# kieranrcampbell/clonealign

Hardware: AMD Instinct MI355X
Metric: ELBO iterations/sec (higher is better)
Workload: dtype f32 variables (contraction: float64 series over gene bins; count-matrix products: int8 MFMA, exact); 1 GPU; synthetic 100000 cells x 5000 genes x 8 clones, K=1, S=1, cell-sharded over 1 GPU(s) (BASELINE.json configs[2]); cells=100000, genes=5000, clones=8, K=1, mc_samples=1, y_storage=u8, y_bytes_per_elem=1, fused_sweep=True, fwd_mfma=True, series_form=True, y_mfma=True, parallelism=single, collective=none, allreduce_doubles_per_train_pass=20764, build_id=9192b4fa1486e0e0

## Files before the change

clonealign_amd/csrc/ca_eng_create.inc:

```

constexpr double CA_ML_STREAM_FIXED_US = 6.6;
constexpr double CA_ML_STREAM_BYTES_PER_US = 5.62e6;
constexpr double CA_ML_MIN_STREAM_US = 45.0;
constexpr int CA_ML_MAX_PER = 4;
struct ca_mom_last_in {
  int slots;
  int n_cu;
  int nb_stream, nb_ovf;
  int ngrp, nred;
  int64_t image_bytes;
};
inline int ca_mom_last_free(const ca_mom_last_in& a) { return std::max(a.slots - a.nb_stream, 0); }
inline int ca_mom_last_free_x(const ca_mom_last_in& a) {
  const int xcd = std::max(a.n_cu / 32, 1);
  return a.slots / xcd - cdiv(a.nb_stream, xcd);
}
inline int ca_mom_last_per(const ca_mom_last_in& a) {
  const int xcd = std::max(a.n_cu / 32, 1), free_x = ca_mom_last_free_x(a);
  if (free_x < 1) return 0;
  return std::max(1, cdiv(a.ngrp, free_x * xcd));
}
inline bool ca_mom_last_pick(const ca_mom_last_in& a) {
  if (a.nb_stream + a.ngrp + a.nred <= a.slots) return false;
  const int per = ca_mom_last_per(a);
// ... 375 lines not shown
                                                 : hipOccupancyMaxActiveBlocksPerMultiprocessor(&per_cu, k_ys_mfma_mom<true>, CA_YM_TB, CA_YS4_LDS_BYTES))
                                 : (h->n_ovf > 0 ? hipOccupancyMaxActiveBlocksPerMultiprocessor(&per_cu, k_ys_mfma_ovf_mom<false>, CA_YM_TB, CA_YS_LDS_BYTES)
                                                 : hipOccupancyMaxActiveBlocksPerMultiprocessor(&per_cu, k_ys_mfma_mom<false>, CA_YM_TB, CA_YS_LDS_BYTES));
    if (oe != hipSuccess) { (void)hipGetLastError(); per_cu = 0; }
    ml.slots = per_cu * h->n_cu; ml.n_cu = h->n_cu;
    ml.nb_stream = h->ys_nrg * h->ys_nseg;
    ml.nb_ovf = h->n_ovf > 0 ? cdiv(Nn, CA_TB) + cdiv(h->n_ovf_chunk, CA_TB / 64) : 0;
    ml.ngrp = h->pws.n_gene_blocks; ml.nred = CA_MOM_NRED;
    ml.image_bytes = h->ys_N64 * h->Gp / (h->ys4 ? 2 : 1);
    h->mom_free_slots = ca_mom_last_free(ml);
    h->mom_last = variantx_on(h, CA_VARX_MOM_LAST, "CA_MOM_LAST_ON") || (variant_on(h, CA_VAR_MOM_LAST, "CA_MOM_LAST") && ca_mom_last_pick(ml));
    if (h->opt.variant_off & CA_VAR_MOM_LAST) h->mom_last = false;
    if (h->mom_last) {
      const int per = ca_mom_last_per(ml);
      h->mom_per = per < 1 ? CA_MOM_PER : std::min(per, CA_ML_MAX_PER);
      h->mom_nred = 2 * CA_MOM_NRED;
      const int lab = (h->opt.reserved[1] & ~0xFF) ? h->opt.reserved[1] >> 8 : 0;
      if (lab & 15) h->mom_per = lab & 15;
      if (lab & 16) h->mom_nred = CA_MOM_NRED;
      h->mom_ovf_first = (lab & 32) != 0;
    }
  }
  h->cell_lean = h->poly && variant_on(h, CA_VAR_CELL_LEAN, "CA_CELL_LEAN");
  h->ride_ok = h->ystore == CA_YSTORE_U8 && K == 1 && D <= 2 && h->fused_ok && !h->c16 && h->fwd_cell && (h->fc_tl == 6 || h->fc_tl == 8 || (h->fc_tl == 2 && h->fc_nbig == 0)) &&
               !h->y_ys && variant_on(h, CA_VAR_Y_RIDE, "CA_Y_RIDE");
  const bool tl1_ok = h->fc_tl == 1 && h->fc_nbig == 0 && !h->c16;
  h->ride_ys = h->y_ys && (!h->ys4 || (h->poly && D == 1 && !h->c16 && !h->s2)) && D <= 2 && h->fused_ok && h->fwd_cell && (h->fc_tl == 6 || tl1_ok || (h->fc_tl == 2 && h->fc_nbig == 0)) &&
               variant_on(h, CA_VAR_Y_RIDE, "CA_Y_RIDE");
  h->yfin_split = h->ride_ys && h->bwd_mfma && h->tail_fuse && variant_on(h, CA_VAR_YFIN_RIDE, "CA_YFIN_RIDE");
  if (h->y_ys && !h->ride_ys) h->async_y = false;
  {
    const int tiles = cdiv(Nn, 16), qb = tiles / std::max(h->n_cu, 1), rb = tiles - qb * h->n_cu;
    h->fwd_bal = h->ride_ys && !h->c16 && !h->s2 && D == 1 && C <= 8 && qb >= 1 && qb <= 6 && h->nk32 >= 96 && h->host_dev && variant_on(h, CA_VAR_FWD_BAL, "CA_FWD_BAL");
    if (h->fwd_bal) {
      h->bal_q = qb; h->bal_r = rb;
      h->bal_nchunk = rb > 0 ? std::min(CA_BAL_MAXCHUNK, h->n_cu / rb) : 0;
      CACK(dalloc(h, &h->bal_xw, std::max<int64_t>(1, (int64_t)rb * h->bal_nchunk * 512)));
    }
  }
  h->s2f = h->s2 && h->fused_ok && h->fwd_cell && (h->fc_tl == 2 || h->fc_tl == 6) && (h->ride_ys || !h->ride_ok) && variant_on(h, CA_VAR_S2_FUSE, "CA_S2_FUSE");
  h->layout_series = h->poly || (h->poly_shape && h->opt.world > 1);
  if (h->layout_series) {
    h->off_y = 3 + C;
    h->off_q = h->off_y + (int64_t)h->Gp * K;
    h->off_x = h->off_q + (int64_t)CA_PL_NB * (CA_PL_R + 2) * 8;
    h->off_g = h->off_x + std::max(h->opt.world, 1);
// ... 93 lines not shown
```

clonealign_amd/csrc/ca_eng_loop.inc:

```
int wait_y(ca_engine* h, bool all) {
  if (all) {
    if (h->y_pending) HIPCK(h, hipStreamWaitEvent(h->stream, h->ev_ydone, 0));
    h->y_pending = false; h->yw_pending = false;
  } else if (h->yw_pending) {
    HIPCK(h, hipStreamWaitEvent(h->stream, h->ev_ywdone, 0));
    h->yw_pending = false;
  }
  return CA_OK;
}

int make_etamax(ca_engine* h) {
  if (h->D > 0) {
    LAUNCH(h, CA_KERNEL_OTHER, hipLaunchKernelGGL(k_vmm_final, dim3(1), dim3(64), 0, h->stream, h->vmm_part, h->vmm, h->ngblk, h->D));
    LAUNCH(h, CA_KERNEL_OTHER, hipLaunchKernelGGL(k_etamax, dim3(cdiv(h->N, CA_TB)), dim3(CA_TB), 0, h->stream, h->F, h->vmm, h->etamax2, h->N, h->D));
  }
  h->em_stale = false;
  return CA_OK;
}
int ensure_etamax(ca_engine* h) {
  if (!h->em_stale) return CA_OK;
  return make_etamax(h);
}

int refresh_derived(ca_engine* h) {
// ... 722 lines not shown
    }
    h->ys_defer_next = h->y_ys && !h->ycache_valid && h->opt.reserved[1] != 3;
    const int yrc = ensure_ycache(h);
    const bool mom_left = h->mom_args != nullptr;
    h->mom_args = nullptr;
    CACK(yrc);
    if (mom_left) { h->err = "internal: the series form's moments were to ride on a count-matrix stream launch that was not made"; return CA_ERR_STATE; }
    h->ys_defer_next = false;
    ca_yfin_args yfin_ride;
    const bool yfin_rides = h->yfin_pending;
    if (yfin_rides) { yfin_ride = yfin_args(h, h->ys_nrg, h->ys_nseg); h->yfin_pending = false; }
    if (moments_aside) HIPCK(h, hipStreamWaitEvent(h->stream, h->ev_poly1, 0));
    CACK(prof_begin(h, CA_KERNEL_FWD));
    ca_small_args ltail = no_small_args();
    const bool sh = is_sharded(h) && h->tail_fuse && yfin_rides;
    if (sh) {
      ltail = small_args(h, h->gene_part, 0, 0.f, nullptr, true);
      ltail.ncblk = h->pws.n_cell_blocks;
      if (h->K > 0) { ltail.yw_part = h->yw_part; ltail.n_yw = h->n_yw; }
      ltail.reduce_only = 1; ltail.host_out = nullptr;
    }
    e = ca_poly_cells(h->stream, &h->pws, h->N, h->C, h->K, &cp, h->alpha_u, h->cell_part, h->dFpart, yfin_rides ? &yfin_ride : nullptr,
                      sh ? &ltail : nullptr, h->poly_xmax_ready ? h->poly_xpart : nullptr, (int)cdiv(h->N, CA_TB), h->F, sh ? h->red + h->off_x : nullptr,
                      h->opt.rank, std::max(h->opt.world, 1), h->cell_lean);
    h->mon_tail_local = sh;
    if (sh) { h->poly_xslot_pending = true; h->poly_xglob_steps = -1; }
    HIPCK(h, e);
    CACK(prof_end(h));
    cell_blocks = h->pws.n_cell_blocks;
    h->poly_fresh = true;
  } else
  if (h->fwd_cell && ride && h->ride_ys) {
    cell_blocks = h->ncblk_f;
    CACK(ys_quant(h));
    ca_ysride_args ya;
    memset(&ya, 0, sizeof(ya));
    ya.Ys = h->Ys; ya.io = ys_io(h); ya.F = h->F; ya.V = h->V; ya.Df = h->D;
    ya.Gp = h->Gp; ya.RS = h->ys_RS; ya.nb_main = h->ys_nrg * h->ys_nseg; ya.nb_y = ya.nb_main;
    ya.ovf = ys_ovf(h);
    ya.nb_y += ya.ovf.nb_rows + ya.ovf.nb_chunks;
    if (h->fwd_bal && !s2f) {
      ca_bal_args ba;
      memset(&ba, 0, sizeof(ba));
      ba.nb = h->n_cu; ba.r = h->bal_r; ba.nchunk = h->bal_nchunk; ba.xw = h->bal_xw;
      cell_blocks = h->n_cu;
      if (++h->bal_tag == 0u) h->bal_tag = 1u;
      ba.tag = h->bal_tag;
// ... 188 lines not shown
```

clonealign_amd/csrc/ca_eng_state.inc:

```
namespace {

thread_local std::string g_last_error;

typedef struct { char internal[128]; } ca_nccl_uid;
typedef void* ca_nccl_comm;
struct RcclApi {
  void* lib = nullptr;
  int (*GetUniqueId)(ca_nccl_uid*) = nullptr;
  int (*CommInitRank)(ca_nccl_comm*, int, ca_nccl_uid, int) = nullptr;
  int (*CommDestroy)(ca_nccl_comm) = nullptr;
  int (*AllReduce)(const void*, void*, size_t, int, int, ca_nccl_comm, hipStream_t) = nullptr;
  const char* (*GetErrorString)(int) = nullptr;
  std::string err;
  bool load() {
    if (lib) return true;
    const char* cands[] = {getenv("CLONEALIGN_RCCL_LIB"), "librccl.so.1", "librccl.so", "/opt/rocm/lib/librccl.so.1",
                           "/opt/rocm/lib/librccl.so"};
    for (const char* c : cands) {
      if (!c || !*c) continue;
      lib = dlopen(c, RTLD_NOW | RTLD_LOCAL);
      if (lib) break;
    }
    if (!lib) { err = std::string("cannot dlopen librccl: ") + dlerror(); return false; }
    GetUniqueId = (decltype(GetUniqueId))dlsym(lib, "ncclGetUniqueId");
// ... 85 lines not shown
  float* eps_dev = nullptr; int64_t eps_cap = 0;
  float *mu32 = nullptr, *Mb = nullptr, *Vs = nullptr, *vmm = nullptr, *vmm_part = nullptr, *etamax2 = nullptr;
  double* gene_part = nullptr; int ngblk = 0;
  float *Zpart = nullptr, *coef = nullptr; double* scratch = nullptr;
  double* cell_part = nullptr; int ncblk = 0;
  float *gpart = nullptr, *dFpart = nullptr; int gsplit = 1, gchunk = 0, csplit = 1; int64_t cchunk = 0; int RG = 4, ntile = 0;
  float *YWpart = nullptr, *YTpart = nullptr, *YW = nullptr; double* ytpsi = nullptr;
  double* red = nullptr; int64_t red_n = 0, off_g = 0, off_y = 0;
  int64_t off_q = 0, off_x = 0;
  bool poly_shape = false, layout_series = false;
  bool mon_tail_local = false;
  bool poly_xslot_pending = false;
  int poly_xglob_steps = -1;
  double* elbo_dev = nullptr; int64_t elbo_cap = 0; double* terms_dev = nullptr;
  double* host_pinned = nullptr;
  bool ycache_valid = false, sums_global = false, sums_started = false;
  std::vector<double> mu_part;
  bool fused_ok = false, look_valid = false; int64_t look_slot = 0; int frow = 8;
  bool carry = false, carry_builtin = false; std::vector<float> carry_eps;
  int64_t n_series = 0, n_series_fallback = 0;
  double *poly_ring = nullptr, *poly_ring_dev = nullptr; uint64_t poly_seq = 0, poly_seq_base = 1, adam_steps = 0, poly_steps_at[16] = {};
  bool mom_ride = false; unsigned mom_tag = 0; const ca_pm_args* mom_args = nullptr;
  bool mom_last = false, mom_ovf_first = false; int mom_free_slots = 0, mom_per = CA_MOM_PER, mom_nred = CA_MOM_NRED;
  bool cell_lean = false;
  bool poly = false, poly_side = false, poly_y_defer = false, poly_fresh = false, poly_df = false ; ca_poly_ws pws; float* poly_zero = nullptr; unsigned char* poly_mem = nullptr;
  float *Mb2 = nullptr, *mu32B = nullptr, *Zpart2 = nullptr; double* gene_partB = nullptr;
  bool y_defer = false;
  bool ride_ok = false;
  bool ride_ys = false;
  bool fold_gsum = false, fold_now = false;
  int64_t hint_A = -1, hint_B = -1, pre_A = -1, pre_B = -1;
  bool pre_valid = false, pre_ok = true, pair_elbo = true;
  double* ee_partB = nullptr;
  double *gene_part_alt = nullptr, *gene_partB_alt = nullptr;
  bool bwd_ready = false; int64_t bwd_slot = -1;
  double* yw_part = nullptr; int n_yw = 0;
  bool yfin_split = false, yfin_pending = false;
  ca_small_args mon_tail;
  bool tail_fuse = true;
  double* host_dev = nullptr;
  unsigned long long host_seq = 0, host_seq_next = 0;
  float* eps_stage = nullptr; size_t eps_stage_bytes = 0;
  hipEvent_t ev_stage = nullptr;
  bool fwd_cell = false; int ncblk_f = 0, fc_tl = 4;
  int fc_nbig = 0;
  bool fwd_mfma = false; int fsplit = 1, fkchunk = 1, nk32 = 1; unsigned short* Mq = nullptr;
// ... 318 lines not shown
```

clonealign_amd/csrc/ca_poly.h:

```cpp
#pragma once
#include <hip/hip_runtime.h>
#include <stddef.h>
#include <stdint.h>

#define CA_PL_R 20
#define CA_PL_NB 32
#define CA_PL_A 2.0
#ifndef CA_PL_NBL
#define CA_PL_NBL 4
#endif

struct ca_poly_hdr { double vlo, delta, xmax; int nb, bad; };
struct ca_poly_ws {
  ca_poly_hdr* hdr; unsigned int* xbits; unsigned int* mflags ; double *tabB, *partB, *tabQ, *Qpart;
  int n_cell_blocks, n_gene_blocks;
};

inline bool ca_poly_ok(int D, int S, int C) { return D == 1 && S == 1 && C >= 3 && C <= 8; }
size_t ca_poly_workspace_bytes(int G, int n_cell_blocks);
void ca_poly_bind(ca_poly_ws* w, void* base, int G, int n_cell_blocks);
hipError_t ca_poly_moments(hipStream_t st, const ca_poly_ws* w, const float* V, const float* F, const float* muA, const float* muB, const float* Lb, int G,
                           int64_t N, int C, unsigned int* bad_word ,
                           double* mirror , double seq, const float* xpart, int nx,
                           const double* xglob , int nglob, double xadd);
hipError_t ca_poly_ranges(hipStream_t st, const ca_poly_ws* w, const float* V, const float* F, int G, int64_t N, double* mirror, double seq, const float* xpart, int nx,
                          const double* xglob, int nglob, double xadd);
hipError_t ca_poly_xslot(hipStream_t st, const float* xpart, int nx, const float* F, int64_t N, double* slots, int rank, int world);
inline bool ca_poly_covers(double xmax, double vlo, double vhi, int steps, double step_bound) {
  const double x = xmax + steps * step_bound, wdt = (vhi - vlo) + 2.0 * steps * step_bound;
  return x == x && wdt == wdt && x * wdt <= 2.0 * CA_PL_A * CA_PL_NB;
}
hipError_t ca_poly_cells(hipStream_t st, const ca_poly_ws* w, int64_t N, int C, int K, const void* cell_ptrs, const float* alpha_u, double* cell_part, float* dF,
                         const void* yfin_args ,
                         const void* local_tail ,
                         const float* xs_part, int xs_n, const float* xs_F, double* xs_slots ,
                         int rank, int world,
                         bool lean );
hipError_t ca_poly_backward(hipStream_t st, const ca_poly_ws* w, const float* V, const float* mu, const float* Lb, int G, int C, double* red_g,
                            const void* small_tail );
```

clonealign_amd/csrc/ca_poly.hip:

```cpp
#include <hip/hip_runtime.h>
#include <stdint.h>

#include <algorithm>
#include <cstring>
#include <type_traits>

#include "ca_poly.h"

namespace ca_series {
#include "ca_kernels.hip.h"

constexpr int R = CA_PL_R, NB = CA_PL_NB;
#include "ca_polymom.hip.h"
constexpr int TB_B = 384;
constexpr int GPB = CA_PM_GPB;

__device__ __forceinline__ float warp_max(float v) {
#pragma unroll
  for (int o = 32; o > 0; o >>= 1) v = fmaxf(v, __shfl_xor(v, o, 64));
  return v;
}
__device__ __forceinline__ float warp_min(float v) {
#pragma unroll
  for (int o = 32; o > 0; o >>= 1) v = fminf(v, __shfl_xor(v, o, 64));
// ... 35 lines not shown
#pragma unroll
    for (int u = 0; u < U; ++u) { const int g = g0_ + u * CA_TB + t; v[u] = V[g < G ? g : G - 1]; }
#pragma unroll
    for (int u = 0; u < U; ++u) { mn = fminf(mn, v[u]); mx = fmaxf(mx, v[u]); }
  }
  mn = warp_min(mn); mx = warp_max(mx);
  if ((t & 63) == 0) { smn[t >> 6] = mn; smx[t >> 6] = mx; }
  __syncthreads();
  if (t == 0) {
    mn = fminf(fminf(smn[0], smn[1]), fminf(smn[2], smn[3]));
    mx = fmaxf(fmaxf(smx[0], smx[1]), fmaxf(smx[2], smx[3]));
    double xmax = nx > 0 ? (double)fmaxf(fmaxf(sxm[0], sxm[1]), fmaxf(sxm[2], sxm[3])) : (double)__uint_as_float(*xbits);
    if (nglob > 0) { xmax = 0.0; for (int r = 0; r < nglob; ++r) xmax = fmax(xmax, xglob[r]); xmax += xadd; }
    *xbits = 0u;
    ca_poly_mirror_store(mirror, seq, xmax, (double)mn, (double)mx);
  }
}

__global__ void __launch_bounds__(TB_B) k_poly_B(ca_pm_args a) {
  __shared__ ca_pm_lds s;
  ca_pm_B_body<TB_B, false>(a, (int)blockIdx.x, 1, blockIdx.x == 0, s);
}

template <int CP, bool LEAN>
__global__ void __launch_bounds__(CA_TB) k_poly_cell(const ca_poly_hdr* __restrict__ hdr, const double* __restrict__ tabB, ca_cell_ptrs p,
                                                     const float* __restrict__ alpha_u, double* __restrict__ cell_part, int64_t N, int C, int K,
                                                     float* __restrict__ dF , double* __restrict__ Qpart , int ncb, ca_yfin_args yfin) {
  if ((int)blockIdx.x >= ncb) {
    const int e = (int)blockIdx.x - ncb;
    const int ncolblk = (yfin.ncol + CA_TB / 64 - 1) / (CA_TB / 64);
    if (e < ncolblk) {
      const int job = e * (CA_TB / 64) + (int)(threadIdx.x >> 6);
      if (job < yfin.ncol) ca_yfin_col_wave(yfin, job);
    } else if (e - ncolblk < yfin.nrow) {
      __shared__ double ca_yfin_sm[CA_TB / 64];
      ca_yfin_row_block(yfin, e - ncolblk, ca_yfin_sm);
    }
    return;
  }
  constexpr int CPB = CA_TB / CP;
  constexpr int RQ = R + 2;
  constexpr int NBR = 4;
  __shared__ double sm[CA_TB];
  __shared__ double la[64];
  __shared__ double s_eb[CPB][NB];
  constexpr int NXK = (RQ + CP - 1) / CP;
  constexpr int XS = LEAN ? NXK * CP : RQ;
  __shared__ double s_xp[CPB][XS];
  __shared__ double s_cf[CPB][8];
  constexpr int NBL = CA_PL_NBL;
  __shared__ double s_tb[NBL][(R + 1) * 16];
  const int nb = hdr->nb;
  ca_log_softmax_alpha(alpha_u, C, la);
  for (int i = threadIdx.x; i < CPB * NB; i += CA_TB) (&s_eb[0][0])[i] = 0.0;
  for (int i = threadIdx.x; i < (nb < NBL ? nb : NBL) * (R + 1) * 16; i += CA_TB) (&s_tb[0][0])[i] = tabB[i];
  __syncthreads();
  const int t = threadIdx.x, c = t % CP, slot = t / CP;
  const double vlo = hdr->vlo, delta = hdr->delta;
  const bool qown = t < RQ * C;
  const int qk = qown ? t / C : 0, qc = qown ? t % C : 0;
  double qa[NBR] = {0.0, 0.0, 0.0, 0.0};
  double* mine = Qpart + (int64_t)blockIdx.x * (NB * RQ * 8);
  if (qown) for (int b = NBR; b < nb; ++b) mine[(b * RQ + qk) * C + qc] = 0.0;
  ca_cell_acc acc = {0.0, 0.0, 0.0, 0.0, 0.0};
  const int64_t ngroups = (N + CPB - 1) / CPB;
  const int cc = c < C ? c : C - 1;
  using pre_t = typename std::conditional<LEAN, ca_cell_pre_lean, ca_cell_pre>::type;
  using x_t = typename std::conditional<LEAN, float, double>::type;
  auto load_pass = [&](int64_t grp, x_t& x_, pre_t& pre_) {
    const int64_t n_ = grp * CPB + slot, nn_ = n_ < N ? n_ : N - 1;
    x_ = (x_t)p.F[nn_];
    pre_.gl = p.glogit[nn_ * C + cc]; pre_.sn = p.s64[nn_]; pre_.Anc = p.A[nn_ * C + cc];
    if constexpr (LEAN) pre_.cn = p.cn[nn_];
  };
  x_t x_next = 0; pre_t pre_next = {};
  if ((int64_t)blockIdx.x < ngroups) load_pass(blockIdx.x, x_next, pre_next);
  [[maybe_unused]] int pass = 0;
  for (int64_t grp = blockIdx.x; grp < ngroups; grp += ncb, ++pass) {
    CA_LAB_CELL_PH(blockIdx.x, pass, 0);
    const int64_t n = grp * CPB + slot;
    const double x = (double)x_next; pre_t pre = pre_next;
    if constexpr (LEAN) pre.x = x;
    if (grp + ncb < ngroups) load_pass(grp + ncb, x_next, pre_next);
    double ZA = 0.0, ZB = 0.0, dZB = 0.0;
// ... 21 lines not shown
#pragma unroll
      for (int j = 0; j < NXK; ++j) keep[j] = 0.0;
#pragma unroll
      for (int k = 0; k < RQ; ++k) { keep[k / CP] = (k % CP == c) ? xk : keep[k / CP]; xk *= x; }
#pragma unroll
      for (int j = 0; j < NXK; ++j) s_xp[slot][j * CP + c] = keep[j];
    } else {
      double xk = 1.0;
      for (int k = 0; k < RQ; ++k) { if (k % CP == c) s_xp[slot][k] = xk; xk *= x; }
    }
    CA_LAB_CELL_PH(blockIdx.x, pass, 2);
    float cff = 0.f;
    ca_cell_fused_group<CP, true, LEAN>(p, la, n, N, C, 1, K, ZA, ZB, acc, &pre, &cff);
    const double cf = (double)cff;
    double df = cf * dZB;
    if constexpr (LEAN) df = ca_dpp_gsum<CP>(df);
    else {
#pragma unroll
    for (int o = CP / 2; o > 0; o >>= 1) df += __shfl_xor(df, o, CP);
    }
    if (c == 0 && n < N) dF[n] = (float)df;
    if (c < 8) s_cf[slot][c] = cf;
    CA_LAB_CELL_PH_AFTER(df, blockIdx.x, pass, 3);
    __syncthreads();
    CA_LAB_CELL_PH(blockIdx.x, pass, 4);
    if (qown) {
      if (nb == 1) {
#pragma unroll 8
        for (int s = 0; s < CPB; ++s) qa[0] += s_cf[s][qc] * s_xp[s][qk] * s_eb[s][0];
      } else {
#pragma unroll 8
        for (int s = 0; s < CPB; ++s) {
          const double w = s_cf[s][qc] * s_xp[s][qk];
          qa[0] += w * s_eb[s][0]; qa[1] += w * s_eb[s][1]; qa[2] += w * s_eb[s][2]; qa[3] += w * s_eb[s][3];
        }
      }
      for (int b = NBR; b < nb; ++b) {
        double a = mine[(b * RQ + qk) * C + qc];
        for (int s = 0; s < CPB; ++s) a += s_cf[s][qc] * s_xp[s][qk] * s_eb[s][b];
        mine[(b * RQ + qk) * C + qc] = a;
      }
    }
    CA_LAB_CELL_PH_AFTER(qa[0], blockIdx.x, pass, 5);
    __syncthreads();
    CA_LAB_CELL_PH(blockIdx.x, pass, 6);
  }
  ca_cell_fused_finish<CP>(acc, sm, cell_part, blockIdx.x, C);
  if (qown) {
#pragma unroll
    for (int b = 0; b < NBR; ++b) if (b < nb) mine[(b * RQ + qk) * C + qc] = qa[b];
  }
}

struct ca_xslot_args { const float* xpart; int nx; const float* F; int64_t N; double* slots; int rank, world; };
__device__ __forceinline__ void ca_poly_xslot_body(const ca_xslot_args& a) {
  __shared__ float sx[CA_TB / 64];
  float ax = 0.f;
  if (a.nx > 0) { for (int i = threadIdx.x; i < a.nx; i += CA_TB) ax = fmaxf(ax, a.xpart[i]); }
  else { for (int64_t i = threadIdx.x; i < a.N; i += CA_TB) { const float v = fabsf(a.F[i]); ax = fmaxf(ax, v == v ? v : INFINITY); } }
  ax = warp_max(ax);
  if ((threadIdx.x & 63) == 0) sx[threadIdx.x >> 6] = ax;
  __syncthreads();
  if ((int)threadIdx.x < a.world) a.slots[threadIdx.x] = (int)threadIdx.x == a.rank ? (double)fmaxf(fmaxf(sx[0], sx[1]), fmaxf(sx[2], sx[3])) : 0.0;
}
__global__ void __launch_bounds__(CA_TB) k_poly_red(const double* __restrict__ part, int nblk, int64_t stride, const ca_poly_hdr* __restrict__ hdr, int per_bin,
                                                    int mode, int C, double* __restrict__ out, unsigned int* __restrict__ xbits, int nred, ca_small_args tail,
                                                    ca_xslot_args xs) {
  if ((int)blockIdx.x >= nred) {
    const int e = (int)blockIdx.x - nred;
    if (e == 0 && tail.enabled) ca_final_small_body(tail);
    else if (xs.slots) ca_poly_xslot_body(xs);
// ... 94 lines not shown
  return hipGetLastError();
}

hipError_t ca_poly_moments(hipStream_t st, const ca_poly_ws* w, const float* V, const float* F, const float* muA, const float* muB, const float* Lb, int G,
                           int64_t N, int C, unsigned int* bad_word, double* mirror, double seq, const float* xpart, int nx, const double* xglob, int nglob, double xadd) {
  if (!xpart) nx = 0;
  if (!xglob) nglob = 0;
  if (nx == 0 && nglob == 0) hipLaunchKernelGGL(k_poly_xmax, dim3((unsigned)std::min<int64_t>(128, (N + 4 * CA_TB - 1) / (4 * CA_TB))), dim3(CA_TB), 0, st, F, N, w->xbits);
  ca_pm_args a;
  memset(&a, 0, sizeof(a));
  a.V = V; a.xbits = w->xbits; a.muA = muA; a.muB = muB; a.Lb = Lb; a.G = G; a.C = C; a.hdr = w->hdr; a.part = w->partB; a.bad_word = bad_word; a.mirror = mirror; a.seq = seq;
  a.xpart = xpart; a.nx = nglob ? 0 : nx; a.xglob = xglob; a.nglob = nglob; a.xadd = xadd;
  hipLaunchKernelGGL(k_poly_B, dim3(w->n_gene_blocks), dim3(TB_B), 0, st, a);
  {
    ca_small_args no_tail; memset(&no_tail, 0, sizeof(no_tail));
    ca_xslot_args no_xs; memset(&no_xs, 0, sizeof(no_xs));
    hipLaunchKernelGGL(k_poly_red, dim3(256), dim3(CA_TB), 0, st, w->partB, w->n_gene_blocks, (int64_t)NB * (R + 1) * 16, w->hdr,
                       (R + 1) * 16, 0, C, w->tabB, w->xbits, 256, no_tail, no_xs);
  }
  return hipGetLastError();
}

hipError_t ca_poly_cells(hipStream_t st, const ca_poly_ws* w, int64_t N, int C, int K, const void* cell_ptrs, const float* alpha_u, double* cell_part, float* dF,
                         const void* yfin_args, const void* local_tail, const float* xs_part, int xs_n, const float* xs_F, double* xs_slots, int rank, int world, bool lean) {
  const ca_cell_ptrs& p = *static_cast<const ca_cell_ptrs*>(cell_ptrs);
  ca_yfin_args yfin;
  if (yfin_args) memcpy(&yfin, yfin_args, sizeof(yfin)); else memset(&yfin, 0, sizeof(yfin));
  int CP = 1;
  while (CP < C) CP <<= 1;
  const int nextra = yfin_args ? cdiv_i(yfin.ncol, CA_TB / 64) + yfin.nrow : 0;
  const dim3 grid(w->n_cell_blocks + nextra);
#define CA_PCELL(CPV, LV) hipLaunchKernelGGL((k_poly_cell<CPV, LV>), grid, dim3(CA_TB), 0, st, w->hdr, w->tabB, p, alpha_u, cell_part, N, C, K, dF, w->Qpart, \
                                         w->n_cell_blocks, yfin)
  if (lean) {
    if (K > 1) return hipErrorInvalidValue;
    if (CP == 4) CA_PCELL(4, true); else CA_PCELL(8, true);
  } else {
    if (CP == 4) CA_PCELL(4, false); else CA_PCELL(8, false);
  }
#undef CA_PCELL
  {
    ca_small_args tail;
    if (local_tail) memcpy(&tail, local_tail, sizeof(tail)); else memset(&tail, 0, sizeof(tail));
    const ca_xslot_args xs = {xs_part, xs_part ? xs_n : 0, xs_F, N, xs_slots, rank, world};
    const int nextra = (tail.enabled || xs_slots) ? 2 : 0;
    hipLaunchKernelGGL(k_poly_red, dim3(256 + nextra), dim3(CA_TB), 0, st, w->Qpart, w->n_cell_blocks, (int64_t)NB * (R + 2) * 8, w->hdr,
                       (R + 2) * C, 1, C, w->tabQ, nullptr, 256, tail, xs);
  }
  return hipGetLastError();
}

hipError_t ca_poly_backward(hipStream_t st, const ca_poly_ws* w, const float* V, const float* mu, const float* Lb, int G, int C, double* red_g, const void* small_tail) {
  ca_small_args tail;
  static_assert(sizeof(ca_small_args) <= 512, "ca_small_args");
  if (small_tail) memcpy(&tail, small_tail, sizeof(tail)); else memset(&tail, 0, sizeof(tail));
  const int ngblk = cdiv_i(G, CA_TB);
  hipLaunchKernelGGL(k_poly_gene, dim3(ngblk + (tail.enabled ? 1 : 0)), dim3(CA_TB), 0, st, w->hdr, w->tabQ, V, mu, Lb, G, C, red_g, tail, ngblk);
  return hipGetLastError();
}

#ifdef CA_LAB
extern "C" int ca_lab_read_cell_stamps(unsigned long long* out, int n_words) {
  return hipMemcpyFromSymbol(out, HIP_SYMBOL(ca_series::ca_lab_stamps4), (size_t)n_words * sizeof(unsigned long long)) == hipSuccess ? 0 : 2;
// ... 3 lines not shown
```

clonealign_amd/csrc/clonealign_hip.hip:

```cpp
#include "clonealign_hip.h"

#include <dlfcn.h>
#include <unistd.h>
#include <hip/hip_runtime.h>

#include <algorithm>
#include <cmath>
#include <cstdio>
#include <cstring>
#include <string>
#include <atomic>
#include <chrono>
#include <thread>
#include <vector>

#include "ca_kernels.hip.h"
#include "ca_poly.h"
#include "philox_host.h"

#include "ca_eng_state.inc"
#include "ca_eng_launch.inc"
#include "ca_eng_reduce.inc"
#include "ca_eng_loop.inc"
#include "ca_eng_ingest.inc"
// ... 291 lines not shown
  if (h->host_ar_buf) hipHostFree(h->host_ar_buf);
  if (h->poly_ring) hipHostFree(h->poly_ring);
  if (h->stream) hipStreamDestroy(h->stream);
  delete h;
  return CA_OK;
}

int ca_get_info(ca_handle h, ca_info* i) {
  if (!h || !i) return CA_ERR_INVALID;
  memset(i, 0, sizeof(*i));
  i->N = h->N; i->G = h->G; i->C = h->C; i->K = h->K; i->P = h->P; i->S = h->S;
  i->y_storage = h->ystore; i->y_bytes_per_elem = h->ybytes; i->y_device_bytes = h->y_dev_bytes; i->device_bytes = h->dev_bytes;
  i->gsplit = h->gsplit; i->csplit = h->csplit; i->n_cu = h->n_cu; i->fused_sweep = h->fused_ok ? 1 : 0;
  i->fwd_mfma = ((h->fused_ok && h->fwd_mfma) || h->pfwd) ? 1 : 0; i->bwd_mfma = h->bwd_mfma ? 1 : 0; i->fsplit = h->fsplit; i->fwd_cell = (h->fused_ok && h->fwd_cell) ? 1 : 0;
  i->y_mfma = h->y_ys ? 2 : 0;
  i->y_stream_bits = h->y_ys ? (h->ys4 ? 4 : 8) : 0;
  i->y_ride = (h->ride_ok || h->ride_ys) ? 1 : 0;
  i->transport = (h->p2p && h->p2p->connected) ? CA_TRANSPORT_P2P : h->comm ? CA_TRANSPORT_RCCL : h->host_ar ? CA_TRANSPORT_HOST : CA_TRANSPORT_NONE;
  i->red_n = h->red_n;
  i->fwd_block_cells = (h->fused_ok && h->fwd_cell) ? 16 * h->fc_tl : 0; i->fwd_blocks_big = h->fc_nbig;
  i->fwd_balanced = h->fwd_bal ? h->bal_q : 0;
  i->fwd_series = h->poly ? 1 : 0; i->series_passes = h->n_series; i->series_fallbacks = h->n_series_fallback;
  i->mom_ride = h->mom_ride ? 1 : 0;
  i->cell_lean = h->cell_lean ? 1 : 0;
  i->mom_last = h->mom_last ? 1 : 0; i->mom_free_slots = h->mom_free_slots;
  i->fold_gsum = (h->fold_gsum && !is_sharded(h)) ? 1 : 0; i->yfin_split = (h->yfin_split && !is_sharded(h)) ? 1 : 0;
  i->update_merge = (h->upd_merge && h->fused_ok && h->fwd_cell && h->K > 0) ? 1 : 0;
  return CA_OK;
}

int ca_stream_busy(ca_handle h, int32_t* busy) {
  if (!h || !busy) return CA_ERR_INVALID;
  const hipError_t q = hipStreamQuery(h->stream);
  if (q != hipSuccess && q != hipErrorNotReady) HIPCK(h, q);
  *busy = q == hipErrorNotReady ? 1 : 0;
  if (q == hipErrorNotReady) (void)hipGetLastError();
  return CA_OK;
}

int ca_synchronize(ca_handle h) {
  if (!h) return CA_ERR_INVALID;
  HIPCK(h, hipSetDevice(h->device));
  CACK(gate_close(h));
  SYNC(h);
  return CA_OK;
}

// ... 439 lines not shown
```

clonealign_amd/engine.py:

```python
import ctypes as C
import os

import numpy as np

_HERE = os.path.dirname(os.path.abspath(__file__))
LIB_PATH = os.path.join(_HERE, "libclonealign_hip.so")

CA_OK = 0
CA_ERR_NAN = 4
CA_INTERRUPTED = 7
CA_ABI_VERSION = 6
P2P_HANDLE_BYTES = 128
CA_F64, CA_F32, CA_I32, CA_U16, CA_U8 = 0, 1, 2, 3, 4
CA_ROW_MAJOR, CA_COL_MAJOR = 0, 1
YSTORE = {"auto": 0, "f32": 1, "u16": 2, "u8": 3}
YSTORE_NAME = {v: k for k, v in YSTORE.items()}
KERNEL_NAMES = ("fwd", "bwd", "ypass", "cell", "other")
VARIANTS = {"fused": 1 << 0, "fwd_mfma": 1 << 1, "fwd_cell": 1 << 2, "bwd_mfma": 1 << 3, "tail_fuse": 1 << 4, "async_y": 1 << 5,
            "pre": 1 << 6, "pair_elbo": 1 << 7, "prep_fast": 1 << 8, "update_merge": 1 << 9, "p2p": 1 << 10, "fold_gsum": 1 << 11, "y_ride": 1 << 12, "ride_seq": 1 << 13, "y_mfma1": 1 << 14, "yfin_ride": 1 << 15, "p2p_ride": 1 << 16, "run_gate": 1 << 17, "s2_fuse": 1 << 18, "fwd_bal": 1 << 19, "bwd_tl3": 1 << 20, "series": 1 << 21, "y4": 1 << 22, "mom_ride": 1 << 23, "cell_lean": 1 << 24, "mom_last": 1 << 25}
VARIANTS_ON = {"y_mfma2": 1 << 0, "async_small": 1 << 1, "y_mfma1": 1 << 2, "fold_always": 1 << 3, "ride_seq": 1 << 4, "p2p_same_device": 1 << 5, "run_fwd": 1 << 6, "bal_tiles": 1 << 7, "series": 1 << 8, "y4": 1 << 9, "mom_last": 1 << 10}
OPT_VERBOSE = 0x80000000
TUNE = {"gsplit": 0, "fsplit": 1, "fc_tl": 2, "fc_nbig": 3, "csplit": 4, "csplit_m": 5, "tr": 6, "rg": 7}
TRANSPORT_NAME = {0: "none", 1: "rccl", 2: "host", 3: "p2p"}

EXPORTS = (
    "ca_abi_version", "ca_build_id", "ca_device_count", "ca_default_options", "ca_create", "ca_destroy", "ca_last_error", "ca_get_info",
    "ca_synchronize", "ca_stream_busy", "ca_comm_unique_id", "ca_comm_init", "ca_p2p_export", "ca_p2p_connect", "ca_p2p_commit", "ca_comm_benchmark", "ca_comm_selftest", "ca_set_host_allreduce", "ca_gamma_init", "ca_elbo", "ca_elbo_terms",
    "ca_step", "ca_gradients", "ca_run", "ca_run_ex", "ca_iterate", "ca_final_elbo", "ca_init_psi_pca", "ca_clone_gene_sums", "ca_get_param", "ca_set_param",
    "ca_get_gradient", "ca_reinit", "ca_get_kernel_times", "ca_reset_kernel_times", "ca_set_profile", "ca_eps_draw", "ca_allele_loglik", "ca_preprocess",
    "ca_group_create", "ca_group_destroy", "ca_group_last_error", "ca_group_get_info", "ca_group_rank_handle", "ca_group_init_psi_pca", "ca_group_gamma_init",
    "ca_group_elbo", "ca_group_step", "ca_group_run_ex", "ca_group_iterate", "ca_group_final_elbo", "ca_group_get_param", "ca_group_reinit",
    "ca_group_clone_gene_sums",
    "ca_create_sparse", "ca_group_create_sparse",
    "ca_fit_mse", "ca_group_fit_mse",
    "ca_logexpr_sums", "ca_group_logexpr_sums",
    "ca_clone_loglik", "ca_group_clone_loglik",
    "ca_project_cells", "ca_group_project_cells",
    "ca_clone_pair_loglik", "ca_group_clone_pair_loglik",
    "ca_simulate_counts", "ca_simulate_kernel_ms",
    "ca_predictive_stats", "ca_predictive_kernel_ms",
)
CA_SPARSE_CSR, CA_SPARSE_CSC = 0, 1
# ... 11 lines not shown
class CaSparse(C.Structure):
    _fields_ = [("kind", C.c_int32), ("val_dtype", C.c_int32), ("index_bytes", C.c_int32), ("on_device", C.c_int32),
                ("nnz", C.c_int64), ("ptr", C.c_void_p), ("idx", C.c_void_p), ("val", C.c_void_p)]


class CaOptions(C.Structure):
    _fields_ = [("learning_rate", C.c_double), ("beta1", C.c_double), ("beta2", C.c_double),
                ("adam_eps", C.c_double), ("seed", C.c_uint64), ("device", C.c_int32),
                ("y_storage", C.c_int32), ("rank", C.c_int32), ("world", C.c_int32), ("profile", C.c_int32),
                ("variant_off", C.c_uint32), ("tune", C.c_int32 * 8), ("variant_on", C.c_uint32),
                ("ride_pattern", C.c_int32), ("comm_timeout_ms", C.c_int32), ("gate_timeout_us", C.c_int32), ("reserved", C.c_int32 * 2)]


class CaInfo(C.Structure):
    _fields_ = [("N", C.c_int64), ("G", C.c_int32), ("C", C.c_int32), ("K", C.c_int32), ("P", C.c_int32),
                ("S", C.c_int32), ("y_storage", C.c_int32), ("y_bytes_per_elem", C.c_int32),
                ("y_device_bytes", C.c_int64), ("device_bytes", C.c_int64), ("gsplit", C.c_int32),
                ("csplit", C.c_int32), ("n_cu", C.c_int32), ("fused_sweep", C.c_int32), ("fwd_mfma", C.c_int32),
                ("bwd_mfma", C.c_int32), ("fsplit", C.c_int32), ("fwd_cell", C.c_int32), ("y_mfma", C.c_int32),
                ("transport", C.c_int32), ("y_ride", C.c_int32), ("red_n", C.c_int64),
                ("fwd_block_cells", C.c_int32), ("fwd_blocks_big", C.c_int32), ("fold_gsum", C.c_int32), ("yfin_split", C.c_int32),
                ("update_merge", C.c_int32), ("fwd_balanced", C.c_int32), ("fwd_series", C.c_int32), ("y_stream_bits", C.c_int32),
                ("series_passes", C.c_int64), ("series_fallbacks", C.c_int64), ("mom_ride", C.c_int32), ("cell_lean", C.c_int32),
                ("mom_last", C.c_int32), ("mom_free_slots", C.c_int32)]


class CaGroupInfo(C.Structure):
    _fields_ = [("world", C.c_int32), ("transport", C.c_int32), ("p2p_status", C.c_int32), ("rccl_status", C.c_int32),
                ("rebuilds", C.c_int32), ("selftest_rounds", C.c_int32), ("N", C.c_int64), ("note", C.c_char * 384)]


class CaPreprocessParams(C.Structure):
    _fields_ = [("min_counts_per_gene", C.c_double), ("min_counts_per_cell", C.c_double),
                ("remove_outlying_genes", C.c_int32), ("remove_genes_same_copy_number", C.c_int32),
                ("nmads", C.c_double), ("max_copy_number", C.c_double)]


HOST_ALLREDUCE_FN = C.CFUNCTYPE(C.c_int, C.c_void_p, C.POINTER(C.c_double), C.c_int64)
POLL_FN = C.CFUNCTYPE(C.c_int, C.c_void_p, C.c_int32, C.c_double)

_lib = None


def load_library(path=None):
    global _lib
    if _lib is not None and path is None:
        return _lib
# ... 858 lines not shown
```

include/clonealign_hip.h:

```cpp
#ifndef CLONEALIGN_HIP_H
#define CLONEALIGN_HIP_H

#include <stdint.h>

#ifdef __cplusplus
extern "C" {
#endif

#define CA_ABI_VERSION 6

typedef struct ca_engine* ca_handle;

enum ca_status {
  CA_OK = 0,
  CA_ERR_INVALID = 1,
  CA_ERR_HIP = 2,
  CA_ERR_NOMEM = 3,
  CA_ERR_NAN = 4,
  CA_ERR_COMM = 5,
  CA_ERR_STATE = 6,
  CA_INTERRUPTED = 7
};

enum ca_dtype { CA_F64 = 0, CA_F32 = 1, CA_I32 = 2, CA_U16 = 3, CA_U8 = 4 };
// ... 26 lines not shown
  CA_VAR_FWD_CELL = 1 << 2,
  CA_VAR_BWD_MFMA = 1 << 3,
  CA_VAR_TAIL_FUSE = 1 << 4,
  CA_VAR_ASYNC_Y = 1 << 5,
  CA_VAR_PRE = 1 << 6,
  CA_VAR_PAIR_ELBO = 1 << 7,
  CA_VAR_PREP_FAST = 1 << 8,
  CA_VAR_UPDATE_MERGE = 1 << 9,
  CA_VAR_P2P_RIDE = 1 << 16,
  CA_VAR_RUN_GATE = 1 << 17,
  CA_VAR_S2_FUSE = 1 << 18,
  CA_VAR_FWD_BAL = 1 << 19,
  CA_VAR_BWD_TL3 = 1 << 20,
  CA_VAR_SERIES = 1 << 21,
  CA_VAR_P2P = 1 << 10,
  CA_VAR_FOLD_GSUM = 1 << 11,
  CA_VAR_Y_RIDE = 1 << 12,
  CA_VAR_Y_MFMA1 = 1 << 14,
  CA_VAR_YFIN_RIDE = 1 << 15,
  CA_VAR_Y4 = 1 << 22,
  CA_VAR_MOM_RIDE = 1 << 23,
  CA_VAR_CELL_LEAN = 1 << 24,
  CA_VAR_MOM_LAST = 1 << 25,
  CA_VAR_RIDE_SEQ = 1 << 13
};
enum ca_variant_on {
  CA_VARX_Y_MFMA2 = 1 << 0,
  CA_VARX_Y_MFMA1 = 1 << 2,
  CA_VARX_FOLD_ALWAYS = 1 << 3,
  CA_VARX_RIDE_SEQ = 1 << 4,
  CA_VARX_P2P_SAME_DEVICE = 1 << 5,
  CA_VARX_RUN_FWD = 1 << 6,
  CA_VARX_BAL_TILES = 1 << 7,
  CA_VARX_SERIES = 1 << 8,
  CA_VARX_Y4 = 1 << 9,
  CA_VARX_MOM_LAST = 1 << 10,
  CA_VARX_ASYNC_SMALL = 1 << 1
};
#define CA_OPT_VERBOSE 0x80000000u
enum ca_tune_id {
  CA_TUNE_GSPLIT = 0, CA_TUNE_FSPLIT = 1, CA_TUNE_FC_TL = 2, CA_TUNE_FC_NBIG = 3, CA_TUNE_CSPLIT = 4, CA_TUNE_CSPLIT_M = 5,
  CA_TUNE_TR = 6, CA_TUNE_RG = 7, CA_TUNE_COUNT = 8
};

typedef struct ca_options {
  double learning_rate;
// ... 24 lines not shown
  int32_t fused_sweep;
  int32_t fwd_mfma;
  int32_t bwd_mfma;
  int32_t fsplit;
  int32_t fwd_cell;
  int32_t y_mfma;
  int32_t transport;
  int32_t y_ride;
  int64_t red_n;
  int32_t fwd_block_cells;
  int32_t fwd_blocks_big;
  int32_t fold_gsum;
  int32_t yfin_split;
  int32_t update_merge;
  int32_t fwd_balanced;
  int32_t fwd_series;
  int32_t y_stream_bits;
  int64_t series_passes;
  int64_t series_fallbacks;
  int32_t mom_ride;
  int32_t cell_lean;
  int32_t mom_last;
  int32_t mom_free_slots;
} ca_info;
enum ca_transport { CA_TRANSPORT_NONE = 0, CA_TRANSPORT_RCCL = 1, CA_TRANSPORT_HOST = 2, CA_TRANSPORT_P2P = 3 };

enum ca_kernel_id {
  CA_KERNEL_FWD = 0,
  CA_KERNEL_BWD = 1,
  CA_KERNEL_YPASS = 2,
  CA_KERNEL_CELL = 3,
  CA_KERNEL_OTHER = 4,
  CA_KERNEL_COUNT = 5
};

int ca_abi_version(void);
const char* ca_build_id(void);
int ca_device_count(int32_t* n);
int ca_default_options(ca_options* opts);

int ca_create(const ca_problem* problem, const ca_options* opts, ca_handle* out);

enum ca_sparse_kind { CA_SPARSE_CSR = 0,
                      CA_SPARSE_CSC = 1 };
typedef struct ca_sparse {
  int32_t kind;
// ... 150 lines not shown
```

Baseline: 9034 iterations/s.

## Accumulate per-cell series moments with f64 MFMA tiles in poly cell kernel

Adds an MFMA variant of the series-form cell kernel. Each wave now accumulates the per-block moment sums (x-power times clone factor times bin weight) as 16x16x4 f64 MFMA tiles, replacing the qown-thread scalar loop and its per-pass __syncthreads. The four waves' tiles are combined through shared memory at block end. Bins beyond the register tile still take the scalar path. The cost is extra shared-memory staging at the finish, plus some wasted MFMA lanes when C is smaller than CP.

```diff
diff --git a/clonealign_amd/csrc/ca_eng_create.inc b/clonealign_amd/csrc/ca_eng_create.inc
--- a/clonealign_amd/csrc/ca_eng_create.inc
+++ b/clonealign_amd/csrc/ca_eng_create.inc
@@ -421,6 +421,7 @@
     }
   }
   h->cell_lean = h->poly && variant_on(h, CA_VAR_CELL_LEAN, "CA_CELL_LEAN");
+  h->cell_mfma = h->poly && variant_on(h, CA_VAR_CELL_MFMA, "CA_CELL_MFMA");
   h->ride_ok = h->ystore == CA_YSTORE_U8 && K == 1 && D <= 2 && h->fused_ok && !h->c16 && h->fwd_cell && (h->fc_tl == 6 || h->fc_tl == 8 || (h->fc_tl == 2 && h->fc_nbig == 0)) &&
                !h->y_ys && variant_on(h, CA_VAR_Y_RIDE, "CA_Y_RIDE");
   const bool tl1_ok = h->fc_tl == 1 && h->fc_nbig == 0 && !h->c16;
diff --git a/clonealign_amd/csrc/ca_eng_loop.inc b/clonealign_amd/csrc/ca_eng_loop.inc
--- a/clonealign_amd/csrc/ca_eng_loop.inc
+++ b/clonealign_amd/csrc/ca_eng_loop.inc
@@ -768,7 +768,7 @@
     }
     e = ca_poly_cells(h->stream, &h->pws, h->N, h->C, h->K, &cp, h->alpha_u, h->cell_part, h->dFpart, yfin_rides ? &yfin_ride : nullptr,
                       sh ? &ltail : nullptr, h->poly_xmax_ready ? h->poly_xpart : nullptr, (int)cdiv(h->N, CA_TB), h->F, sh ? h->red + h->off_x : nullptr,
-                      h->opt.rank, std::max(h->opt.world, 1), h->cell_lean);
+                      h->opt.rank, std::max(h->opt.world, 1), h->cell_lean, h->cell_mfma);
     h->mon_tail_local = sh;
     if (sh) { h->poly_xslot_pending = true; h->poly_xglob_steps = -1; }
     HIPCK(h, e);
diff --git a/clonealign_amd/csrc/ca_eng_state.inc b/clonealign_amd/csrc/ca_eng_state.inc
--- a/clonealign_amd/csrc/ca_eng_state.inc
+++ b/clonealign_amd/csrc/ca_eng_state.inc
@@ -131,6 +131,7 @@
   double *poly_ring = nullptr, *poly_ring_dev = nullptr; uint64_t poly_seq = 0, poly_seq_base = 1, adam_steps = 0, poly_steps_at[16] = {};
   bool mom_ride = false; unsigned mom_tag = 0; const ca_pm_args* mom_args = nullptr;
   bool mom_last = false, mom_ovf_first = false; int mom_free_slots = 0, mom_per = CA_MOM_PER, mom_nred = CA_MOM_NRED;
+  bool cell_mfma = false;
   bool cell_lean = false;
   bool poly = false, poly_side = false, poly_y_defer = false, poly_fresh = false, poly_df = false ; ca_poly_ws pws; float* poly_zero = nullptr; unsigned char* poly_mem = nullptr;
   float *Mb2 = nullptr, *mu32B = nullptr, *Zpart2 = nullptr; double* gene_partB = nullptr;
diff --git a/clonealign_amd/csrc/ca_poly.h b/clonealign_amd/csrc/ca_poly.h
--- a/clonealign_amd/csrc/ca_poly.h
+++ b/clonealign_amd/csrc/ca_poly.h
@@ -35,6 +35,7 @@
                          const void* local_tail ,
                          const float* xs_part, int xs_n, const float* xs_F, double* xs_slots ,
                          int rank, int world,
-                         bool lean );
+                         bool lean ,
+                         bool mfma );
 hipError_t ca_poly_backward(hipStream_t st, const ca_poly_ws* w, const float* V, const float* mu, const float* Lb, int G, int C, double* red_g,
                             const void* small_tail );
diff --git a/clonealign_amd/csrc/ca_poly.hip b/clonealign_amd/csrc/ca_poly.hip
--- a/clonealign_amd/csrc/ca_poly.hip
+++ b/clonealign_amd/csrc/ca_poly.hip
@@ -81,7 +81,7 @@
   ca_pm_B_body<TB_B, false>(a, (int)blockIdx.x, 1, blockIdx.x == 0, s);
 }
 
-template <int CP, bool LEAN>
+template <int CP, bool LEAN, bool MFMA>
 __global__ void __launch_bounds__(CA_TB) k_poly_cell(const ca_poly_hdr* __restrict__ hdr, const double* __restrict__ tabB, ca_cell_ptrs p,
                                                      const float* __restrict__ alpha_u, double* __restrict__ cell_part, int64_t N, int C, int K,
                                                      float* __restrict__ dF , double* __restrict__ Qpart , int ncb, ca_yfin_args yfin) {
@@ -118,7 +118,18 @@
   const double vlo = hdr->vlo, delta = hdr->delta;
   const bool qown = t < RQ * C;
   const int qk = qown ? t / C : 0, qc = qown ? t % C : 0;
-  double qa[NBR] = {0.0, 0.0, 0.0, 0.0};
+  [[maybe_unused]] double qa[NBR] = {0.0, 0.0, 0.0, 0.0};
+  using qtile_t = __attribute__((ext_vector_type(4))) double;
+  constexpr int BPT = 16 / CP;
+  constexpr int NCT = NBR / BPT;
+  constexpr int KST = 64 / CP / 4;
+  static_assert(CP == 4 || CP == 8, "the MFMA gather's column map");
+  static_assert(CA_TB == 256, "four waves: each owns a quarter of a pass's cells, and the block's end adds four waves' tiles");
+  [[maybe_unused]] qtile_t qm[2][NCT];
+#pragma unroll
+  for (int j = 0; j < NCT; ++j) { qm[0][j] = qtile_t{0.0, 0.0, 0.0, 0.0}; qm[1][j] = qtile_t{0.0, 0.0, 0.0, 0.0}; }
+  const int wv = t >> 6, mrow = t & 15, mk = (t >> 4) & 3;
+  const int mcl = mrow % CP, mbl = mrow / CP;
   double* mine = Qpart + (int64_t)blockIdx.x * (NB * RQ * 8);
   if (qown) for (int b = NBR; b < nb; ++b) mine[(b * RQ + qk) * C + qc] = 0.0;
   ca_cell_acc acc = {0.0, 0.0, 0.0, 0.0, 0.0};
@@ -186,6 +197,39 @@
     if (c == 0 && n < N) dF[n] = (float)df;
     if (c < 8) s_cf[slot][c] = cf;
     CA_LAB_CELL_PH_AFTER(df, blockIdx.x, pass, 3);
+    if constexpr (MFMA) {
+      __builtin_amdgcn_fence(__ATOMIC_RELEASE, "wavefront"); __builtin_amdgcn_wave_barrier(); __builtin_amdgcn_fence(__ATOMIC_ACQUIRE, "wavefront");
+#pragma unroll
+      for (int s = 0; s < KST; ++s) {
+        const int cell = wv * (64 / CP) + s * 4 + mk;
+        const double a0 = s_xp[cell][mrow];
+        const double a1 = s_xp[cell][16 + mrow < XS ? 16 + mrow : XS - 1];
+        const double cfv = s_cf[cell][mcl];
+#pragma unroll
+        for (int j = 0; j < NCT; ++j) {
+          if (j == 0 || nb > j * BPT) {
+            const double bv = cfv * s_eb[cell][j * BPT + mbl];
+            qm[0][j] = __builtin_amdgcn_mfma_f64_16x16x4f64(a0, bv, qm[0][j], 0, 0, 0);
+            qm[1][j] = __builtin_amdgcn_mfma_f64_16x16x4f64(a1, bv, qm[1][j], 0, 0, 0);
+          }
+        }
+      }
+      if (nb > NBR) {
+        __syncthreads();
+        if (qown) {
+          for (int b = NBR; b < nb; ++b) {
+            double a = mine[(b * RQ + qk) * C + qc];
+            for (int s = 0; s < CPB; ++s) a += s_cf[s][qc] * s_xp[s][qk] * s_eb[s][b];
+            mine[(b * RQ + qk) * C + qc] = a;
+          }
+        }
+        __syncthreads();
+      } else {
+        __builtin_amdgcn_fence(__ATOMIC_RELEASE, "wavefront"); __builtin_amdgcn_wave_barrier(); __builtin_amdgcn_fence(__ATOMIC_ACQUIRE, "wavefront");
+      }
+      CA_LAB_CELL_PH_AFTER(qm[0][0][0], blockIdx.x, pass, 4);
+      continue;
+    }
     __syncthreads();
     CA_LAB_CELL_PH(blockIdx.x, pass, 4);
     if (qown) {
@@ -210,7 +254,33 @@
     CA_LAB_CELL_PH(blockIdx.x, pass, 6);
   }
   ca_cell_fused_finish<CP>(acc, sm, cell_part, blockIdx.x, C);
-  if (qown) {
+  if constexpr (MFMA) {
+    constexpr int QW = RQ * NBR * CP;
+    static_assert(CPB * NB >= QW && CPB * XS >= QW && NBL * (R + 1) * 16 >= QW, "a wave's tiles fit each of the three arrays");
+    double* const p1 = &s_eb[0][0], * const p2 = &s_xp[0][0], * const p3 = &s_tb[0][0];
+    double* const pw = wv == 1 ? p1 : (wv == 2 ? p2 : p3);
+#pragma unroll
+    for (int i = 0; i < 2; ++i)
+#pragma unroll
+      for (int j = 0; j < NCT; ++j)
+#pragma unroll
+        for (int r = 0; r < 4; ++r) {
+          const int k = 16 * i + 4 * r + mk;
+          if (wv > 0 && k < RQ) pw[k * (NBR * CP) + j * 16 + mrow] = qm[i][j][r];
+        }
+    __syncthreads();
+    if (wv == 0) {
+#pragma unroll
+      for (int i = 0; i < 2; ++i)
+#pragma unroll
+        for (int j = 0; j < NCT; ++j)
+#pragma unroll
+          for (int r = 0; r < 4; ++r) {
+            const int k = 16 * i + 4 * r + mk, col = j * 16 + mrow, b = j * BPT + mbl;
+            if (k < RQ && b < nb && mcl < C) mine[(b * RQ + k) * C + mcl] = ((qm[i][j][r] + p1[k * (NBR * CP) + col]) + p2[k * (NBR * CP) + col]) + p3[k * (NBR * CP) + col];
+          }
+    }
+  } else if (qown) {
 #pragma unroll
     for (int b = 0; b < NBR; ++b) if (b < nb) mine[(b * RQ + qk) * C + qc] = qa[b];
   }
@@ -351,7 +421,7 @@
 }
 
 hipError_t ca_poly_cells(hipStream_t st, const ca_poly_ws* w, int64_t N, int C, int K, const void* cell_ptrs, const float* alpha_u, double* cell_part, float* dF,
-                         const void* yfin_args, const void* local_tail, const float* xs_part, int xs_n, const float* xs_F, double* xs_slots, int rank, int world, bool lean) {
+                         const void* yfin_args, const void* local_tail, const float* xs_part, int xs_n, const float* xs_F, double* xs_slots, int rank, int world, bool lean, bool mfma) {
   const ca_cell_ptrs& p = *static_cast<const ca_cell_ptrs*>(cell_ptrs);
   ca_yfin_args yfin;
   if (yfin_args) memcpy(&yfin, yfin_args, sizeof(yfin)); else memset(&yfin, 0, sizeof(yfin));
@@ -359,7 +429,8 @@
   while (CP < C) CP <<= 1;
   const int nextra = yfin_args ? cdiv_i(yfin.ncol, CA_TB / 64) + yfin.nrow : 0;
   const dim3 grid(w->n_cell_blocks + nextra);
-#define CA_PCELL(CPV, LV) hipLaunchKernelGGL((k_poly_cell<CPV, LV>), grid, dim3(CA_TB), 0, st, w->hdr, w->tabB, p, alpha_u, cell_part, N, C, K, dF, w->Qpart, \
+#define CA_PCELL(CPV, LV) do { if (mfma) CA_PCELL_(CPV, LV, true); else CA_PCELL_(CPV, LV, false); } while (0)
+#define CA_PCELL_(CPV, LV, MV) hipLaunchKernelGGL((k_poly_cell<CPV, LV, MV>), grid, dim3(CA_TB), 0, st, w->hdr, w->tabB, p, alpha_u, cell_part, N, C, K, dF, w->Qpart, \
                                          w->n_cell_blocks, yfin)
   if (lean) {
     if (K > 1) return hipErrorInvalidValue;
@@ -368,6 +439,7 @@
     if (CP == 4) CA_PCELL(4, false); else CA_PCELL(8, false);
   }
 #undef CA_PCELL
+#undef CA_PCELL_
   {
     ca_small_args tail;
     if (local_tail) memcpy(&tail, local_tail, sizeof(tail)); else memset(&tail, 0, sizeof(tail));
diff --git a/clonealign_amd/csrc/clonealign_hip.hip b/clonealign_amd/csrc/clonealign_hip.hip
--- a/clonealign_amd/csrc/clonealign_hip.hip
+++ b/clonealign_amd/csrc/clonealign_hip.hip
@@ -337,7 +337,7 @@
   i->fwd_balanced = h->fwd_bal ? h->bal_q : 0;
   i->fwd_series = h->poly ? 1 : 0; i->series_passes = h->n_series; i->series_fallbacks = h->n_series_fallback;
   i->mom_ride = h->mom_ride ? 1 : 0;
-  i->cell_lean = h->cell_lean ? 1 : 0;
+  i->cell_lean = h->cell_lean ? 1 : 0; i->cell_mfma = h->cell_mfma ? 1 : 0;
   i->mom_last = h->mom_last ? 1 : 0; i->mom_free_slots = h->mom_free_slots;
   i->fold_gsum = (h->fold_gsum && !is_sharded(h)) ? 1 : 0; i->yfin_split = (h->yfin_split && !is_sharded(h)) ? 1 : 0;
   i->update_merge = (h->upd_merge && h->fused_ok && h->fwd_cell && h->K > 0) ? 1 : 0;
diff --git a/clonealign_amd/engine.py b/clonealign_amd/engine.py
--- a/clonealign_amd/engine.py
+++ b/clonealign_amd/engine.py
@@ -17,7 +17,7 @@
 YSTORE_NAME = {v: k for k, v in YSTORE.items()}
 KERNEL_NAMES = ("fwd", "bwd", "ypass", "cell", "other")
 VARIANTS = {"fused": 1 << 0, "fwd_mfma": 1 << 1, "fwd_cell": 1 << 2, "bwd_mfma": 1 << 3, "tail_fuse": 1 << 4, "async_y": 1 << 5,
-            "pre": 1 << 6, "pair_elbo": 1 << 7, "prep_fast": 1 << 8, "update_merge": 1 << 9, "p2p": 1 << 10, "fold_gsum": 1 << 11, "y_ride": 1 << 12, "ride_seq": 1 << 13, "y_mfma1": 1 << 14, "yfin_ride": 1 << 15, "p2p_ride": 1 << 16, "run_gate": 1 << 17, "s2_fuse": 1 << 18, "fwd_bal": 1 << 19, "bwd_tl3": 1 << 20, "series": 1 << 21, "y4": 1 << 22, "mom_ride": 1 << 23, "cell_lean": 1 << 24, "mom_last": 1 << 25}
+            "pre": 1 << 6, "pair_elbo": 1 << 7, "prep_fast": 1 << 8, "update_merge": 1 << 9, "p2p": 1 << 10, "fold_gsum": 1 << 11, "y_ride": 1 << 12, "ride_seq": 1 << 13, "y_mfma1": 1 << 14, "yfin_ride": 1 << 15, "p2p_ride": 1 << 16, "run_gate": 1 << 17, "s2_fuse": 1 << 18, "fwd_bal": 1 << 19, "bwd_tl3": 1 << 20, "series": 1 << 21, "y4": 1 << 22, "mom_ride": 1 << 23, "cell_lean": 1 << 24, "mom_last": 1 << 25, "cell_mfma": 1 << 26}
 VARIANTS_ON = {"y_mfma2": 1 << 0, "async_small": 1 << 1, "y_mfma1": 1 << 2, "fold_always": 1 << 3, "ride_seq": 1 << 4, "p2p_same_device": 1 << 5, "run_fwd": 1 << 6, "bal_tiles": 1 << 7, "series": 1 << 8, "y4": 1 << 9, "mom_last": 1 << 10}
 OPT_VERBOSE = 0x80000000
 TUNE = {"gsplit": 0, "fsplit": 1, "fc_tl": 2, "fc_nbig": 3, "csplit": 4, "csplit_m": 5, "tr": 6, "rg": 7}
@@ -75,7 +75,7 @@
                 ("fwd_block_cells", C.c_int32), ("fwd_blocks_big", C.c_int32), ("fold_gsum", C.c_int32), ("yfin_split", C.c_int32),
                 ("update_merge", C.c_int32), ("fwd_balanced", C.c_int32), ("fwd_series", C.c_int32), ("y_stream_bits", C.c_int32),
                 ("series_passes", C.c_int64), ("series_fallbacks", C.c_int64), ("mom_ride", C.c_int32), ("cell_lean", C.c_int32),
-                ("mom_last", C.c_int32), ("mom_free_slots", C.c_int32)]
+                ("mom_last", C.c_int32), ("mom_free_slots", C.c_int32), ("cell_mfma", C.c_int32)]
 
 
 class CaGroupInfo(C.Structure):
diff --git a/include/clonealign_hip.h b/include/clonealign_hip.h
--- a/include/clonealign_hip.h
+++ b/include/clonealign_hip.h
@@ -72,6 +72,7 @@
   CA_VAR_MOM_RIDE = 1 << 23,
   CA_VAR_CELL_LEAN = 1 << 24,
   CA_VAR_MOM_LAST = 1 << 25,
+  CA_VAR_CELL_MFMA = 1 << 26,
   CA_VAR_RIDE_SEQ = 1 << 13
 };
 enum ca_variant_on {
@@ -142,6 +143,7 @@
   int32_t cell_lean;
   int32_t mom_last;
   int32_t mom_free_slots;
+  int32_t cell_mfma;
 } ca_info;
 enum ca_transport { CA_TRANSPORT_NONE = 0, CA_TRANSPORT_RCCL = 1, CA_TRANSPORT_HOST = 2, CA_TRANSPORT_P2P = 3 };
 
```

Result: faster. 9340 iterations/s (median of 6 runs) (+3.4%).
